# czbiohub-sf/yogo

Measured on AMD Instinct MI355X. Metric: training images/sec (772x1032 gray), higher is better.
Workload: dtype bf16; 1 GPU; BASELINE configs[2]: full train step (fwd+loss+bwd+clamp+AdamW), base_model, 772x1032x1 uint8, 7 classes; per_gpu_batch=128, global_batch=128, parallelism=dp1

## Files before the change

### include/yogo_hip.h

```cpp
#ifndef YOGO_HIP_H
#define YOGO_HIP_H

#include <stddef.h>

#ifdef __cplusplus
extern "C" {
#endif

typedef void* yogo_stream_t;

const char* yogo_hip_last_error(void);
int yogo_hip_abi_version(void);
int yogo_hip_launch_log(int enable);
int yogo_hip_launch_log_read(char* buf, size_t cap, size_t* needed);


int yogo_conv_packed_bytes(int Cin, int Cout, int ksize, int stride, int mode, size_t* bytes);
int yogo_conv_pack_f32(const float* w_oihw, float* packed, int Cin, int Cout, int ksize, int stride, int mode,
                       yogo_stream_t stream);
int yogo_conv2d_fwd_stats_shape(int B, int Cin, int Cout, int IH, int IW, int ksize, int stride, int* rows, int* mpad);
int yogo_conv2d_fwd_f32(const float* in, const float* packed, const float* bias, float* out, float* out_pre,
                        const float* chan_scale, float* stats_part, int B, int Cin, int Cout, int IH, int IW, int ksize,
                        int stride, int act, yogo_stream_t stream);
int yogo_conv2d_dgrad_f32(const float* dy, const float* packed_dgrad, float* dx, const float* act_ref, int ref_act,
// ... 12 lines not shown
                          int IW, int stride, yogo_stream_t stream);

int yogo_bn_finalize(const float* part, int rows, int row_stride, int C, long long count, float eps, float momentum,
                     float* mean_out, float* invstd_out, float* running_mean, float* running_var,
                     long long* num_batches_tracked, yogo_stream_t stream);
int yogo_bn_apply_act(const float* z, float* y, const float* mean, const float* invstd_or_var, int stat_is_var, float eps,
                      const float* gamma, const float* beta, int B, int C, int HW, int act, yogo_stream_t stream);
int yogo_bn_invstd(const float* var, float eps, float* invstd, int C, yogo_stream_t stream);
int yogo_bn_bwd_rows(int B, int HW, int* rows);
int yogo_bn_bwd(const float* g, const float* z, float* dz, const float* mean, const float* invstd, const float* gamma,
                const float* beta, int act, float* dgamma, float* dbeta, float* part, float* sums, int B, int C, int HW,
                int training, float clip, yogo_stream_t stream);
int yogo_partials_reduce(float* part, int rows, int N, float clip, float* out, yogo_stream_t stream);
int yogo_channel_sum(const float* g, int B, int C, int HW, float clip, float* out, yogo_stream_t stream);

int yogo_decode_fwd(const float* raw, float* out, const float* cxs, const float* cys, int B, int P, int Sy, int Sx,
                    float anchor_w, float anchor_h, float width_multiplier, float height_multiplier, int inference,
                    yogo_stream_t stream);
int yogo_decode_bwd(const float* raw, const float* out, const float* gout, float* graw, int B, int P, int Sy, int Sx,
                    int inference, yogo_stream_t stream);

int yogo_decode_bwd_bf16(const float* raw, const float* out, const float* gout, void* graw8c, int B, int P, int Sy, int Sx,
                         int inference, yogo_stream_t stream);

int yogo_loss_workspace_bytes(int B, int Sy, int Sx, size_t* bytes);
int yogo_loss_fwd_bwd(const float* pred, const float* label, float* grad, float* loss_out, void* workspace, int B, int P,
                      int Sy, int Sx, float no_obj_weight, float iou_weight, float classify_weight, float label_smoothing,
                      yogo_stream_t stream);

int yogo_decode_loss_bwd_bf16(const float* raw, const float* label, const float* cxs, const float* cys, void* graw8c, float* loss_out,
                              void* workspace, int B, int P, int Sy, int Sx, float anchor_w, float anchor_h, float width_multiplier,
                              float height_multiplier, float no_obj_weight, float iou_weight, float classify_weight,
                              float label_smoothing, yogo_stream_t stream);

int yogo_format_preds_workspace_bytes(int B, int Sy, int Sx, size_t* bytes);
int yogo_format_preds_batched(const float* pred, float* out_rows, long long* out_cells, int* out_count, void* workspace,
                              int B, int P, int Sy, int Sx, int cap, double obj_thresh, double iou_thresh, int box_format,
                              double min_class_confidence_threshold, yogo_stream_t stream);
int yogo_decode_format_preds_batched(const float* raw, const float* cxs, const float* cys, float* out_rows, long long* out_cells,
                                     int* out_count, void* workspace, int B, int P, int Sy, int Sx, int cap, float anchor_w,
                                     float anchor_h, float width_multiplier, float height_multiplier, int inference,
                                     double obj_thresh, double iou_thresh, int box_format, double min_class_confidence_threshold,
                                     yogo_stream_t stream);
int yogo_head1x1_decode_fwd_bf16(const void* x, const void* packed, const float* bias, float* out, const float* cxs, const float* cys,
                                 int B, int Cin, int P, int Sy, int Sx, float anchor_w, float anchor_h, float width_multiplier,
                                 float height_multiplier, int inference, yogo_stream_t stream);

int yogo_match_workspace_bytes(int B, int Sy, int Sx, int cap, size_t* bytes);
int yogo_match_preds_labels_batched(const float* rows, const int* counts, const float* labels, int* meta, int* pair_label,
                                    int* pair_pred, int* un_label, int* un_pred, float* lab_out, void* workspace, int B, int P, int Sy,
                                    int Sx, int cap, yogo_stream_t stream);
int yogo_match_gather(const float* rows, const float* lab_out, const int* meta, const int* pair_label, const int* pair_pred,
                      const int* un_label, const int* un_pred, float* preds, float* labels, float* missed, float* extra, int B, int P,
                      int cap, long long K, long long Km, long long Ke, yogo_stream_t stream);
int yogo_metrics_state_layout(int C, int T, int nbins, long long* offsets);
int yogo_metrics_accumulate(const float* rows, const float* lab_out, const int* meta, const int* pair_label, const int* pair_pred,
                            const int* un_label, const int* un_pred, const double* roc_thresholds, int T, const double* cal_edges,
                            int nbins, long long* acc, double* bin_conf, double* partial, float* map_rows, long long map_cap, int B,
                            int P, int cap, yogo_stream_t stream);

int yogo_pred_sink_state_layout(int C, long long* offsets);
int yogo_pred_sink_workspace_bytes(int B, size_t* bytes);
int yogo_pred_sink_append(const float* rows, const int* counts, int B, int cap, int P, int mode, int count_classes,
                          long long first_img_id, int img_h, int img_w, long long* state, float* arena, long long arena_cap,
                          int* img_counts, long long img_cap, void* workspace, yogo_stream_t stream);

// ... 134 lines not shown
```

### yogo_amd/csrc/decode_loss.hip

```cpp
#include "common.h"

#define MAX_CLASSES 64

__device__ __forceinline__ float sigmoidf_(float x) { return 1.0f / (1.0f + expf(-x)); }

__global__ __launch_bounds__(256) void decode_fwd_kernel(const float* __restrict__ raw, float* __restrict__ out,
                                                         const float* __restrict__ cxs, const float* __restrict__ cys,
                                                         float inv_sx, float inv_sy, float anchor_w, float anchor_h,
                                                         float wmul, float hmul, int P, int cells, int inference) {
  const int b = blockIdx.y;
  const int cell = blockIdx.x * 256 + threadIdx.x;
  if (cell >= cells) return;
  const float* r = raw + (size_t)b * P * cells + cell;
  float* o = out + (size_t)b * P * cells + cell;
  const float t0 = r[0], t1 = r[(size_t)cells], t2 = r[(size_t)2 * cells], t3 = r[(size_t)3 * cells], t4 = r[(size_t)4 * cells];
  o[0] = inv_sx * sigmoidf_(t0) + cxs[cell];
  o[(size_t)cells] = inv_sy * sigmoidf_(t1) + cys[cell];
  o[(size_t)2 * cells] = anchor_w * expf(fminf(t2, 80.f)) * wmul;
  o[(size_t)3 * cells] = anchor_h * expf(fminf(t3, 80.f)) * hmul;
  o[(size_t)4 * cells] = sigmoidf_(t4);
  const int C = P - 5;
  if (inference) {
    float mx = -INFINITY;
    for (int c = 0; c < C; ++c) mx = fmaxf(mx, r[(size_t)(5 + c) * cells]);
    float sum = 0.f;
    for (int c = 0; c < C; ++c) sum += expf(r[(size_t)(5 + c) * cells] - mx);
    for (int c = 0; c < C; ++c) o[(size_t)(5 + c) * cells] = expf(r[(size_t)(5 + c) * cells] - mx) / sum;
  } else {
    for (int c = 0; c < C; ++c) o[(size_t)(5 + c) * cells] = r[(size_t)(5 + c) * cells];
  }
}

__global__ __launch_bounds__(256) void decode_bwd_kernel(const float* __restrict__ raw, const float* __restrict__ out,
// ... 311 lines not shown
        if (ch < p.P) {
          if (ch == 0) v = g0 * (p.inv_sx * (s0 * (1.f - s0)));
          else if (ch == 1) v = g1 * (p.inv_sy * (s1 * (1.f - s1)));
          else if (ch == 2) v = t2 <= 80.f ? g2 * pw : 0.f;
          else if (ch == 3) v = t3 <= 80.f ? g3 * ph : 0.f;
          else if (ch == 4) v = gobj * (po * (1.f - po));
          else if (m != 0.f) {
            const int c = ch - 5;
            const float sm = expf(r[(size_t)ch * cells] - lse);
            v = scl * (sm - (c == tgt ? (1.f - ls) : 0.f) - ls / (float)C);
          }
        }
        u[j] = (__bf16)v;
      }
      p.g8[((size_t)b * p.Pb + kb) * cells + cell] = __builtin_bit_cast(dl_u32x4, u);
    }
  }
  l_iou = wave_sum(l_iou);
  l_obj = wave_sum(l_obj);
  l_cls = wave_sum(l_cls);
  const int lane = threadIdx.x & 63, wave = threadIdx.x >> 6;
  if (lane == 0) {
    sh[0][wave] = l_iou;
    sh[1][wave] = l_obj;
    sh[2][wave] = l_cls;
  }
  __syncthreads();
  if (threadIdx.x < 3) {
    const int k = threadIdx.x;
    p.part[((size_t)b * gridDim.x + blockIdx.x) * 3 + k] = sh[k][0] + sh[k][1] + sh[k][2] + sh[k][3];
  }
}

__global__ __launch_bounds__(256) void yogo_loss_finalize_kernel(const float* __restrict__ part, int rows, float iou_weight,
                                                                 float classify_weight, float inv_batch,
                                                                 float* __restrict__ out) {
  __shared__ double sh[3][4];
  double s[3] = {0.0, 0.0, 0.0};
  for (int r = threadIdx.x; r < rows; r += 256)
    for (int k = 0; k < 3; ++k) s[k] += (double)part[(size_t)r * 3 + k];
  const int lane = threadIdx.x & 63, wave = threadIdx.x >> 6;
  for (int k = 0; k < 3; ++k) {
    s[k] = wave_sum_d(s[k]);
    if (lane == 0) sh[k][wave] = s[k];
  }
  __syncthreads();
  if (threadIdx.x == 0) {
    const float iou = (float)(iou_weight * (sh[0][0] + sh[0][1] + sh[0][2] + sh[0][3]) * inv_batch);
    const float obj = (float)((sh[1][0] + sh[1][1] + sh[1][2] + sh[1][3]) * inv_batch);
    const float cls = (float)(classify_weight * (sh[2][0] + sh[2][1] + sh[2][2] + sh[2][3]) * inv_batch);
    out[0] = obj + iou + cls;
    out[1] = iou;
    out[2] = obj;
    out[3] = cls;
  }
}

extern "C" int yogo_decode_fwd(const float* raw, float* out, const float* cxs, const float* cys, int B, int P, int Sy,
                               int Sx, float anchor_w, float anchor_h, float width_multiplier, float height_multiplier,
                               int inference, hipStream_t stream) {
  YOGO_CHECK_ARG(raw && out && cxs && cys, "decode_fwd: null pointer");
  YOGO_CHECK_ARG(B >= 0 && P > 5 && P - 5 <= MAX_CLASSES && Sy > 0 && Sx > 0 && B <= 65535, "decode_fwd: bad shape");
  if (B == 0) return YOGO_OK;
  const int cells = Sy * Sx;
  yogo_launch_log("decode_fwd_kernel | B=%d cells=%d P=%d inference=%d", B, cells, P, inference);
  hipLaunchKernelGGL(decode_fwd_kernel, dim3(cdiv(cells, 256), B), dim3(256), 0, stream, raw, out, cxs, cys,
// ... 34 lines not shown
}

extern "C" int yogo_loss_fwd_bwd(const float* pred, const float* label, float* grad, float* loss_out, void* workspace,
                                 int B, int P, int Sy, int Sx, float no_obj_weight, float iou_weight, float classify_weight,
                                 float label_smoothing, hipStream_t stream) {
  YOGO_CHECK_ARG(pred && label && grad && loss_out && workspace, "loss_fwd_bwd: null pointer");
  YOGO_CHECK_ARG(B > 0 && B <= 65535 && P > 5 && P - 5 <= MAX_CLASSES && Sy > 0 && Sx > 0, "loss_fwd_bwd: bad shape");
  LossParams p{};
  p.pred = pred; p.label = label; p.grad = grad; p.part = reinterpret_cast<float*>(workspace);
  p.B = B; p.P = P; p.cells = Sy * Sx;
  p.no_obj_weight = no_obj_weight; p.iou_weight = iou_weight; p.classify_weight = classify_weight;
  p.label_smoothing = label_smoothing; p.inv_batch = 1.0f / (float)B;
  const int nb = cdiv(p.cells, 256);
  hipLaunchKernelGGL(yogo_loss_kernel, dim3(nb, B), dim3(256), 0, stream, p);
  hipLaunchKernelGGL(yogo_loss_finalize_kernel, dim3(1), dim3(256), 0, stream, p.part, B * nb, iou_weight, classify_weight,
                     p.inv_batch, loss_out);
  YOGO_CHECK_LAUNCH("loss_fwd_bwd");
  return YOGO_OK;
}

extern "C" int yogo_decode_loss_bwd_bf16(const float* raw, const float* label, const float* cxs, const float* cys, void* graw8c, float* loss_out,
                                         void* workspace, int B, int P, int Sy, int Sx, float anchor_w, float anchor_h, float width_multiplier,
                                         float height_multiplier, float no_obj_weight, float iou_weight, float classify_weight,
                                         float label_smoothing, hipStream_t stream) {
  YOGO_CHECK_ARG(raw && label && cxs && cys && graw8c && loss_out && workspace, "decode_loss_bwd_bf16: null pointer");
  YOGO_CHECK_ARG(B > 0 && B <= 65535 && P > 5 && P - 5 <= MAX_CLASSES && Sy > 0 && Sx > 0, "decode_loss_bwd_bf16: bad shape");
  FusedParams p{};
  p.raw = raw; p.label = label; p.cxs = cxs; p.cys = cys; p.g8 = reinterpret_cast<dl_u32x4*>(graw8c); p.part = reinterpret_cast<float*>(workspace);
  p.B = B; p.P = P; p.Pb = ((P + 15) / 16) * 2; p.cells = Sy * Sx;
  p.inv_sx = (float)(1.0 / Sx); p.inv_sy = (float)(1.0 / Sy); p.anchor_w = anchor_w; p.anchor_h = anchor_h; p.wmul = width_multiplier; p.hmul = height_multiplier;
  p.no_obj_weight = no_obj_weight; p.iou_weight = iou_weight; p.classify_weight = classify_weight; p.label_smoothing = label_smoothing;
  p.inv_batch = 1.0f / (float)B;
  const int nb = cdiv(p.cells, 256);
  hipLaunchKernelGGL(decode_loss_bwd_bf16_kernel, dim3(nb, B), dim3(256), 0, stream, p);
  hipLaunchKernelGGL(yogo_loss_finalize_kernel, dim3(1), dim3(256), 0, stream, p.part, B * nb, iou_weight, classify_weight, p.inv_batch, loss_out);
  YOGO_CHECK_LAUNCH("decode_loss_bwd_bf16");
  return YOGO_OK;
}
```

### yogo_amd/engine.py

```python
from __future__ import annotations

import threading
import weakref
from dataclasses import dataclass, field
from typing import Dict, List, Optional, Tuple

import torch
from torch import nn

from yogo_amd import _hip

ACT_NONE, ACT_LEAKY, ACT_SILU = 0, 1, 2


@dataclass
class Layer:
    conv: nn.Conv2d
    bn: Optional[nn.BatchNorm2d] = None
    act: int = ACT_NONE
    drop: Optional[nn.Dropout2d] = None

    @property
    def cin(self) -> int:
        return self.conv.in_channels
# ... 293 lines not shown
                Lp, Sp = self.layers[i - 1], saved[i - 1]
                ref_act = Lp.act
                if Lp.bn is not None:
                    act_ref, ref_act = None, ACT_NONE
                elif Lp.act == ACT_SILU:
                    act_ref = Sp.pre
                    if act_ref is None:
                        raise RuntimeError("yogo_amd: missing saved pre-activation for a SiLU block")
                elif Lp.act == ACT_LEAKY:
                    act_ref = Sp.y
                else:
                    act_ref = None
                dx = torch.empty(B, L.cin, IH, IW, dtype=torch.float32, device=dev)
                pk = self._packed(i, 1)
                mw_tag = 20 if L.s == 2 else (4 if L.cin > 64 else (2 if L.cin > 32 else 1))
                self._tick("dgrad", i, 2.0 * B * L.cout * L.cin * L.k * L.k * OH * OW, mw=mw_tag)
                _hip.call("yogo_conv2d_dgrad_f32", g, pk, dx, act_ref, ref_act, Sp.mask, B, L.cin, L.cout, IH, IW, L.k, L.s, st)
                self._tock()
                g = dx
        bb = self.backbone_ref()
        return [grads.get(id(p)) for p in bb.parameters()]



def _blocks(c: int) -> int:
    return ((c + 15) // 16) * 2


_FUSE_LAYER0_BWD = True
_L0_NO_Z = True
_WGRAD_DEFER_REDUCE = True
_L01_FUSE_BWD = True
_HEAD_BN_FUSE = True


def _packed_bf16(eng: Engine, i: int, mode: int) -> torch.Tensor:
    L = eng.layers[i]
    w = L.conv.weight
    key = (i, 10 + mode)
    buf = _pack_hit(eng, key, w)
    if buf is not None:
        return buf
    nbytes = _hip.query_size("yogo_conv_bf16_packed_bytes", L.cin, L.cout, L.k, mode)
    buf = torch.empty(nbytes, dtype=torch.uint8, device=w.device)
    _hip.call("yogo_conv_bf16_pack", _f32(w.detach()), None, buf, L.cin, L.cout, L.k, mode, _hip.stream_ptr())
    eng._pack[key] = (w._version, w.data_ptr(), buf)
    return buf


def _pack_all_bf16(eng: Engine) -> None:
    jobs = [(i, mode) for i in range(1, len(eng.layers)) for mode in (0, 2 if (eng.layers[i].s == 2 and eng.layers[i].k == 3) else 1)]
    ws = [eng.layers[i].conv.weight for i, _ in jobs]
    if any(w.dtype != torch.float32 or not w.is_contiguous() for w in ws) or not jobs:
        return
    if all(_pack_hit(eng, (i, 10 + m), w) is not None for (i, m), w in zip(jobs, ws)):
        return
    dev = ws[0].device
    key = tuple(w.data_ptr() for w in ws)
    st = eng._pack_multi
    if st is None or st[0] != key:
        bufs, rows, blk = [], [], 0
        for (i, mode), w in zip(jobs, ws):
            L = eng.layers[i]
            buf = torch.empty(_hip.query_size("yogo_conv_bf16_packed_bytes", L.cin, L.cout, L.k, mode), dtype=torch.uint8, device=dev)
            bufs.append(buf)
            rows.append([w.data_ptr(), 0, buf.data_ptr(), L.cin, L.cout, L.k, mode, blk])
# ... 97 lines not shown
        pk = _packed_bf16(eng, i, 0)
        nbytes = B * (_blocks(L.cin) * 8 * H * W * 2 + (L.cout * OH * OW * 4 if last else _blocks(L.cout) * 8 * OH * OW * 2))
        eng._tick("fwd", i, 2.0 * B * L.cout * L.cin * L.k * L.k * OH * OW, mw=34 if (L.cout > 64 and L.s == 1) else (35 if (L.cout > 64 and L.cin > 64 and L.k == 3) else 30), nbytes=nbytes)
        if L.act == ACT_SILU and not has_bn:
            S.pre = torch.empty_like(out8)
            _hip.call("yogo_conv2d_fwd_bf16_pre", cur, pk, bias, out8, S.pre, mask, B, L.cin, L.cout, H, W, L.k, L.s, fused_act, st)
        elif L.act == ACT_LEAKY and not has_bn and not last:
            S.signs = torch.empty(_hip.query_size("yogo_bf16_signs_bytes", B, L.cout, OH, OW), dtype=torch.uint8, device=dev)
            _hip.call("yogo_conv2d_fwd_bf16_signs", cur, pk, bias, out8, S.signs, mask, B, L.cin, L.cout, H, W, L.k, L.s, fused_act, st)
        else:
            _hip.call("yogo_conv2d_fwd_bf16", cur, pk, bias, out8, out32, mask, None, B, L.cin, L.cout, H, W, L.k, L.s, fused_act, st)
        eng._tock()
    if not has_bn:
        S.y = out32 if last else out8
        return S.y
    bn = L.bn
    gamma, beta = _bn_affine(L, dev)
    y = torch.empty_like(out8)
    if bn_train:
        if i > 0:
            rows, mpad = _hip.query_ints("yogo_bn_bwd_bf16_rows", 1, B, OH * OW)[0], L.cout
            stats = torch.empty(rows * mpad * 2, dtype=torch.float32, device=dev)
            _hip.call("yogo_bn_stats_bf16", out8, stats, B, L.cout, OH * OW, st)
        mean, invstd = _bn_finalize(eng, L, "yogo_bn_finalize", stats, rows, mpad, count=B * OH * OW, dev=dev, st=st)
    else:
        invstd = torch.empty(L.cout, dtype=torch.float32, device=dev)
        _hip.call("yogo_bn_invstd", bn.running_var, float(bn.eps), invstd, L.cout, st)
        mean = bn.running_mean
    _hip.call("yogo_bn_apply_act_bf16", out8, y, mean, invstd, 0, float(bn.eps), gamma, beta, B, L.cout, OH * OW, L.act, st)
    S.mean, S.invstd, S.bn_train, S.z, S.y = mean, invstd, bn_train, out8, y
    return y


def forward_bf16_train(eng: Engine, x: torch.Tensor) -> Tuple[torch.Tensor, List[Saved]]:
    _check_bf16_train_input(eng, x)
    dev, st, B = x.device, _hip.stream_ptr(), x.shape[0]
    _pack_all_bf16(eng)
    masks = _dropout_masks(eng, B, dev)
    cur = x.contiguous() if x.dtype == torch.uint8 else _f32(x)
    H, W = int(cur.shape[2]), int(cur.shape[3])
    saved: List[Saved] = []
    n = len(eng.layers)
    for i, L in enumerate(eng.layers):
        OH, OW = L.out_hw(H, W)
        if OH <= 0 or OW <= 0:
            raise RuntimeError(f"yogo_amd: image too small at layer {i}")
        last = i == n - 1
        has_bn = L.bn is not None
        if L.act == ACT_SILU and not has_bn and (i == 0 or last):
            raise RuntimeError("yogo_amd: bf16 training of a first / last SiLU block without BatchNorm is not implemented (use fp32)")
        bias = _f32(L.conv.bias.detach()) if L.conv.bias is not None else None
        S = Saved(x_in=cur, mask=masks.get(i))
        bn_train = has_bn and (L.bn.training or L.bn.running_mean is None)
        if (i == 0 and has_bn and S.mask is None and not last and cur.dtype == torch.uint8
                and _hip.lib().yogo_conv_first_mfma_supported(0, L.cin, L.cout, H, W, L.s)):
            cur = _first_mfma_fwd_bf16(eng, L, S, bias, bn_train, B, H, W, st)
        else:
            cur = _layer_fwd_bf16(eng, i, L, S, bias, bn_train, last, B, H, W, st)
        saved.append(S)
        H, W = OH, OW
    return cur, saved


def backward_bf16_train(eng: Engine, saved: List[Saved], graw: torch.Tensor,
                        grad_out: Optional[Dict[int, torch.Tensor]] = None, on_layer=None,
                        trace: Optional[dict] = None, flush_layers=None, stop_at: int = 0) -> List[Optional[torch.Tensor]]:
    n = len(eng.layers)
    if not 0 <= stop_at < n:
        raise ValueError(f"yogo_amd: stop_at {stop_at} is not a layer of this {n}-layer network")
    st, dev, clip = _hip.stream_ptr(), graw.device, float(eng.clip)
    grads: Dict[int, torch.Tensor] = {}

    def dst(param: torch.Tensor) -> torch.Tensor:
        if grad_out is not None and id(param) in grad_out:
            return grad_out[id(param)]
        return torch.empty(param.shape, dtype=torch.float32, device=dev)

    queued_ws: List[torch.Tensor] = []
    wq = _wgrad_queue() if (_WGRAD_DEFER_REDUCE and (on_layer is None or flush_layers is not None)) else None
    flush_at = frozenset(flush_layers) if flush_layers is not None else frozenset()
    if wq is not None:
        _hip.call("yogo_wgrad_reduce_queue_reset", wq)
    if graw.dtype == torch.bfloat16 and graw.ndim == 5:
        g = graw
        B = g.shape[0]
    else:
        graw = _f32(graw)
        B, P, Sy, Sx = graw.shape
        g = torch.empty(B, _blocks(P), Sy, Sx, 8, dtype=torch.bfloat16, device=dev)
        _hip.call("yogo_nchw_f32_to_bf16_8c", graw, g, B, P, Sy * Sx, st)

    def bn_backward(L, S, g, head_g, OH, OW):
        gamma, beta = _bn_affine(L, dev)
        dgamma, dbeta = _bn_grad_dst(L.bn, dst, grads, L.cout, dev)
        rows = _hip.query_ints("yogo_bn_bwd_bf16_rows", 1, B, OH * OW)[0]
        part = torch.empty(rows * L.cout * 2, dtype=torch.float32, device=dev)
        sums = torch.empty(2 * L.cout, dtype=torch.float32, device=dev)
        if head_g is not None:
            dz = torch.empty(B, _blocks(L.cout), OH, OW, 8, dtype=torch.bfloat16, device=dev)
# ... 92 lines not shown
        head_below = bool(_HEAD_BN_FUSE and i == n - 1 and Lp is not None and i - 1 > 0 and L.k == 1 and L.s == 1 and L.cout <= 16
                          and Lp.bn is not None and Lp.cout % 16 == 0 and g.shape[1] == 2)
        act_ref, ref_act = None, ACT_NONE
        if Lp is not None and Lp.bn is None and Lp.act != ACT_NONE:
            act_ref, ref_act = (Sp.y if Lp.act == ACT_LEAKY else Sp.pre), Lp.act
        if trace is not None and g is not None and head_g is None:
            trace[("g", i)] = g.clone()
        if L.bn is not None and not fuse0:
            g, head_g = bn_backward(L, S, g, head_g, OH, OW), None
            if trace is not None:
                trace[("dz", i)] = g.clone()
        dw = dst(L.conv.weight)
        db = dst(L.conv.bias) if L.conv.bias is not None else None
        if fuse0:
            wgrad_first_bn(L, S, g, fused01, dw, IH, IW)
        elif fuse01:
            fused01 = wgrad_dgrad_first(L, S, g, dw, db, IH, IW, OH, OW)
        elif i == 0:
            wgrad_first(L, S, g, dw, db, IH, IW)
        else:
            wgrad(i, L, S, g, dw, db, IH, IW, OH, OW)
        if db is not None:
            grads[id(L.conv.bias)] = db
        grads[id(L.conv.weight)] = dw
        if on_layer is not None:
            if wq is not None and i in flush_at:
                _hip.call("yogo_wgrad_reduce_flush", wq, st)
            on_layer(i)
        if fuse01:
            g = None
        elif head_below:
            head_g = (g, _f32(L.conv.weight.detach()).reshape(L.cout, L.cin), L.cout)
        elif i > stop_at:
            g = dgrad(i, L, g, Sp, act_ref, ref_act, IH, IW, OH, OW)
    if wq is not None:
        _hip.call("yogo_wgrad_reduce_flush", wq, st)
    bb = eng.backbone_ref()
    return [grads.get(id(p)) for p in bb.parameters()]


_WGRAD_QUEUE = None


def _wgrad_queue() -> int:
    global _WGRAD_QUEUE
    if _WGRAD_QUEUE is None:
        import ctypes
        h = ctypes.c_void_p(0)
        _hip.call("yogo_wgrad_reduce_queue_create", ctypes.addressof(h))
        _WGRAD_QUEUE = int(h.value)
    return _WGRAD_QUEUE


_ENGINES: "weakref.WeakKeyDictionary[nn.Module, Engine]" = weakref.WeakKeyDictionary()


def get_engine(backbone: nn.Sequential) -> Engine:
    eng = _ENGINES.get(backbone)
    if eng is None:
        eng = Engine(backbone)
        _ENGINES[backbone] = eng
    return eng


class _BackboneFn(torch.autograd.Function):
    @staticmethod
    def forward(ctx, x, backbone, *params):
# ... 224 lines not shown
```

### yogo_amd/train.py

```python
from __future__ import annotations

import ctypes
import math
from typing import Dict, List, Optional, Tuple

import torch
import torch.distributed as dist

from yogo_amd import _hip
from yogo_amd.engine import get_engine
from yogo_amd.model import YOGO
from yogo_amd.yogo_loss import YOGOLoss

_FUSED_DECODE_LOSS = True


def cosine_lr(step: int, base_lr: float, t_max: int, eta_min: float) -> float:
    return eta_min + (base_lr - eta_min) * (1 + math.cos(math.pi * step / t_max)) / 2


class FlatParams:

    def __init__(self, module: torch.nn.Module):
        self.params: List[torch.nn.Parameter] = [p for p in module.parameters()]
# ... 215 lines not shown
            if icnt is not None:
                _hip.call("yogo_comm_broadcast_flat", self._rccl, icnt, icnt.numel() * 8, src, st)
        else:
            dist.broadcast(flat, src=src, group=self.pg)
            if icnt is not None:
                dist.broadcast(icnt, src=src, group=self.pg)
        off = 0
        for b in fl:
            n = b.numel()
            b.copy_(flat[off:off + n].view(b.shape).to(b.dtype))
            off += n
        off = 0
        for b in cnt:
            n = b.numel()
            b.copy_(icnt[off:off + n].view(b.shape).to(b.dtype))
            off += n
        self.engine.generation += 1

    @torch.no_grad()
    def step(self, imgs: torch.Tensor, labels: torch.Tensor) -> torch.Tensor:
        m = self.model
        _hip.require_cuda(imgs, "imgs")
        _hip.require_cuda(labels, "labels")
        with torch.cuda.device(imgs.device):
            st = _hip.stream_ptr()
            eng = self.engine
            eng.clip = m._clip
            self.flat.check_homed()
            if imgs.ndim == 3:
                imgs = imgs[None]
            if not imgs.is_floating_point() and imgs.dtype != torch.uint8:
                imgs = imgs.float()
            if self.half:
                from yogo_amd.engine import backward_bf16_train, forward_bf16_train

                raw, saved = forward_bf16_train(eng, imgs)
                if self.trace is not None:
                    self.trace["saved"], self.trace["raw"] = saved, raw
            else:
                raw, saved = eng.forward(imgs, need_grad=True)
            B, P, Sy, Sx = raw.shape
            aw, ah, wm, hm = m._decode_scalars()
            cxs, cys = _hip.grid_buffers(m._Cxs, m._Cys, Sy, Sx, raw.device)
            L = self.loss
            out = torch.empty(4, dtype=torch.float32, device=raw.device)
            ws = torch.empty(_hip.query_size("yogo_loss_workspace_bytes", B, Sy, Sx) // 4, dtype=torch.float32, device=raw.device)
            lab = labels if (labels.dtype == torch.float32 and labels.is_contiguous()) else labels.contiguous().float()
            hook = self._on_layer_done if self.world > 1 else None
            flush = (self.split_layer,) if hook is not None else None
            lw = (float(L.no_obj_weight), float(L.iou_weight), float(L.classify_weight), float(L.label_smoothing))

            def decode_and_loss():
                pred, gpred = torch.empty_like(raw), torch.empty_like(raw)
                _hip.call("yogo_decode_fwd", raw, pred, cxs, cys, B, P, Sy, Sx, aw, ah, wm, hm, int(bool(m.inference)), st)
                _hip.call("yogo_loss_fwd_bwd", pred, lab, gpred, out, ws, B, P, Sy, Sx, *lw, st)
                return pred, gpred

            g8 = torch.empty(B, ((P + 15) // 16) * 2, Sy, Sx, 8, dtype=torch.bfloat16, device=raw.device) if self.half else None
            if self.half and not m.inference and _FUSED_DECODE_LOSS:
                _hip.call("yogo_decode_loss_bwd_bf16", raw, lab, cxs, cys, g8, out, ws, B, P, Sy, Sx, aw, ah, wm, hm, *lw, st)
                backward_bf16_train(eng, saved, g8, grad_out=self.flat.grad_views, on_layer=hook, trace=self.trace, flush_layers=flush)
            elif self.half:
                pred, gpred = decode_and_loss()
                _hip.call("yogo_decode_bwd_bf16", raw, pred, gpred, g8, B, P, Sy, Sx, int(bool(m.inference)), st)
                backward_bf16_train(eng, saved, g8, grad_out=self.flat.grad_views, on_layer=hook, trace=self.trace, flush_layers=flush)
            else:
                pred, gpred = decode_and_loss()
                graw = torch.empty_like(raw)
                _hip.call("yogo_decode_bwd", raw, pred, gpred, graw, B, P, Sy, Sx, int(bool(m.inference)), st)
                eng.backward(saved, graw, grad_out=self.flat.grad_views, on_layer=hook)
            started = self.split_off if (self.overlap and self._pending) else self.flat.total
            self.exchange_begin(0, started)
            scale = self.exchange_end()
            lr = self.current_lr()
            self.global_step += 1
            _hip.call("yogo_adamw_step", self.flat.flat, self.flat.grad, self.flat.exp_avg, self.flat.exp_avg_sq, self.flat.total,
                      self.global_step, lr, self.betas[0], self.betas[1], self.eps, self.wd, scale, st)
            eng.invalidate_packed()
            self.last_loss = out
            return out

    def loss_components(self) -> Dict[str, float]:
        v = self.last_loss.cpu().tolist()
        return {"loss": v[0], "iou_loss": v[1], "objectness_loss": v[2], "classification_loss": v[3]}
```

Measured before the change: 11160 images/s.

## Fuse head 1x1 conv, decode, loss and head dgrad into one sweep kernel

Adds a persistent kernel that, for the final 1x1 head layer, computes the head conv with MFMA, decodes, evaluates the YOGO loss and its gradient, and applies the head dgrad multiplied by the leaky activation derivative in a single pass over each pixel tile. It also has an optional path that accumulates weight gradients in the same pass. The forward pass stops before the head, and the backward pass takes the precomputed head dx. The aim is to remove the separate head forward, decode/loss, and dgrad launches along with their intermediate global memory round trips. In exchange the kernel carries heavy register and LDS pressure, and it only handles restricted shapes (P up to 16, Cin up to 128).

```diff
diff --git a/include/yogo_hip.h b/include/yogo_hip.h
--- a/include/yogo_hip.h
+++ b/include/yogo_hip.h
@@ -68,6 +68,14 @@
                               void* workspace, int B, int P, int Sy, int Sx, float anchor_w, float anchor_h, float width_multiplier,
                               float height_multiplier, float no_obj_weight, float iou_weight, float classify_weight,
                               float label_smoothing, yogo_stream_t stream);
+
+int yogo_head_sweep_bf16_supported(int Cin, int P, int ksize, int stride, int Sy, int Sx, int B);
+int yogo_head_sweep_bf16_rows(int B, int Sy, int Sx, int* rows);
+int yogo_head_sweep_bf16_workspace_bytes(int B, int Cin, int P, int Sy, int Sx, size_t* bytes);
+int yogo_head_sweep_bf16(const void* y6, const void* packed, const float* bias, const float* label, const float* cxs, const float* cys,
+                         float* raw, void* g8, void* g6, float* loss_out, void* loss_ws, void* wpart, int B, int Cin, int P, int Sy,
+                         int Sx, float anchor_w, float anchor_h, float width_multiplier, float height_multiplier, float no_obj_weight,
+                         float iou_weight, float classify_weight, float label_smoothing, yogo_stream_t stream);
 
 int yogo_format_preds_workspace_bytes(int B, int Sy, int Sx, size_t* bytes);
 int yogo_format_preds_batched(const float* pred, float* out_rows, long long* out_cells, int* out_count, void* workspace,
diff --git a/yogo_amd/csrc/decode_loss.hip b/yogo_amd/csrc/decode_loss.hip
--- a/yogo_amd/csrc/decode_loss.hip
+++ b/yogo_amd/csrc/decode_loss.hip
@@ -1,4 +1,5 @@
 #include "common.h"
+#include <mutex>
 
 #define MAX_CLASSES 64
 
@@ -376,6 +377,337 @@
   }
 }
 
+typedef float dl_f32x16 __attribute__((ext_vector_type(16)));
+typedef float dl_f32x4 __attribute__((ext_vector_type(4)));
+typedef __bf16 dl_bf16x4 __attribute__((ext_vector_type(4)));
+#define HS_MAXP 16
+#define HS_WAVE_LDS 10240
+
+struct HeadSweepParams {
+  const dl_u32x4* y6;
+  const dl_u32x4* wp;
+  const float* bias;
+  const float* label;
+  const float *cxs, *cys;
+  float* raw;
+  dl_u32x4* g8;
+  dl_u32x4* g6;
+  float* part;
+  float* wpart;
+  int B, P, cells, nb, units, upb;
+  float inv_sx, inv_sy, anchor_w, anchor_h, wmul, hmul;
+  float no_obj_weight, iou_weight, classify_weight, label_smoothing, inv_batch;
+};
+
+__device__ __forceinline__ int hs_off(int row, int ch) { return 256 * row + 16 * (ch ^ (((row & 3) << 2) | ((row >> 2) & 3))); }
+
+__device__ __forceinline__ dl_bf16x8 hs_tr8(const unsigned char* a0, const unsigned char* a1) {
+  typedef dl_bf16x4 __attribute__((address_space(3))) * lds_v4;
+  const dl_bf16x4 lo = __builtin_amdgcn_ds_read_tr16_b64_v4bf16((lds_v4)a0);
+  const dl_bf16x4 hi = __builtin_amdgcn_ds_read_tr16_b64_v4bf16((lds_v4)a1);
+  return __builtin_shufflevector(lo, hi, 0, 1, 2, 3, 4, 5, 6, 7);
+}
+
+template <int NK, bool WG>
+__global__ __launch_bounds__(256, 2) void decode_loss_bwd_bf16_kernel(const HeadSweepParams p) {
+  constexpr int OOB = (int)0x80000000u;
+  constexpr int KB = 2 * NK, NM = (NK + 1) / 2, CIN = 16 * NK;
+  __shared__ __attribute__((aligned(16))) unsigned char lds[WG ? 4 * HS_WAVE_LDS : 16];
+  __shared__ float sh[2][3][4];
+  const int tid = threadIdx.x, lane = tid & 63, l31 = lane & 31, half = lane >> 5, l15 = lane & 15, g4 = lane >> 4;
+  const int wave = __builtin_amdgcn_readfirstlane(tid >> 6);
+  unsigned char* yimg = lds + wave * HS_WAVE_LDS;
+  unsigned char* gimg = yimg + 8192;
+  const int cells = p.cells, cells16 = cells * 16, P = p.P, C = P - 5;
+  __shared__ dl_u32x4 wlds[KB * 32];
+  for (int e = tid; e < KB * 32; e += 256) wlds[e] = p.wp[e];
+  float bs[8];
+#pragma unroll
+  for (int i = 0; i < 8; ++i) {
+    const int ch = 8 * (i >> 2) + 4 * half + (i & 3);
+    bs[i] = (p.bias != nullptr && ch < P) ? p.bias[ch] : 0.f;
+  }
+  dl_bf16x8 Wd[NM];
+  {
+    const __bf16* w16 = reinterpret_cast<const __bf16*>(p.wp);
+    const int q = l31 >> 3, h = (l31 >> 2) & 1, t = l31 & 3;
+#pragma unroll
+    for (int m = 0; m < NM; ++m) {
+      const int cin = 8 * (4 * m + 2 * (q >> 1) + h) + 4 * (q & 1) + t;
+#pragma unroll
+      for (int j = 0; j < 8; ++j) {
+        const int pch = 8 * half + j;
+        Wd[m][j] = (cin < CIN && pch < P) ? w16[(((cin >> 3) * 32 + pch) << 3) + (cin & 7)] : (__bf16)0.f;
+      }
+    }
+  }
+  dl_bf16x8 ones;
+#pragma unroll
+  for (int j = 0; j < 8; ++j) ones[j] = (__bf16)1.f;
+  dl_f32x4 accW[NK], accB = {0.f, 0.f, 0.f, 0.f};
+#pragma unroll
+  for (int c = 0; c < NK; ++c) accW[c] = dl_f32x4{0.f, 0.f, 0.f, 0.f};
+  const int trq = l15 >> 2, trp = l15 & 3;
+
+  __syncthreads();
+  const int u_end = min(p.units, (int)(blockIdx.x + 1) * p.upb);
+  int par = 0;
+  for (int u = blockIdx.x * p.upb; u < u_end; ++u, par ^= 1) {
+    const int b = u / p.nb, blk = u - b * p.nb;
+    const int pxw = blk * 256 + wave * 64;
+    const int px = pxw + lane;
+    const bool valid = px < cells;
+    const auto rs_in = __builtin_amdgcn_make_buffer_rsrc((void*)(p.y6 + (size_t)b * KB * cells), (short)0, KB * cells16, 0x00020000);
+    dl_u32x4 Bq[2][NK];
+    bool ov[2];
+    int pxt[2];
+#pragma unroll
+    for (int T = 0; T < 2; ++T) {
+      pxt[T] = pxw + 32 * T + l31;
+      ov[T] = pxt[T] < cells;
+      const int v0 = ov[T] ? (half * cells + pxt[T]) * 16 : OOB;
+#pragma unroll
+      for (int kc = 0; kc < NK; ++kc) Bq[T][kc] = __builtin_bit_cast(dl_u32x4, __builtin_amdgcn_raw_buffer_load_b128(rs_in, v0, (2 * kc) * cells16, 0));
+    }
+    dl_f32x16 acc[2];
+#pragma unroll
+    for (int T = 0; T < 2; ++T)
+#pragma unroll
+      for (int r = 0; r < 16; ++r) acc[T][r] = 0.f;
+#pragma unroll
+    for (int kc = 0; kc < NK; ++kc) {
+      const dl_bf16x8 a = __builtin_bit_cast(dl_bf16x8, wlds[(2 * kc + half) * 32 + l31]);
+      acc[0] = __builtin_amdgcn_mfma_f32_32x32x16_bf16(a, __builtin_bit_cast(dl_bf16x8, Bq[0][kc]), acc[0], 0, 0, 0);
+      acc[1] = __builtin_amdgcn_mfma_f32_32x32x16_bf16(a, __builtin_bit_cast(dl_bf16x8, Bq[1][kc]), acc[1], 0, 0, 0);
+    }
+    float r[HS_MAXP];
+#pragma unroll
+    for (int i = 0; i < 8; ++i) {
+      const float own = (half == 0 ? acc[0][i] : acc[1][i]) + bs[i];
+      const float snd = (half == 0 ? acc[1][i] : acc[0][i]) + bs[i];
+      const float rcv = __shfl_xor(snd, 32, 64);
+      const int cha = 8 * (i >> 2) + (i & 3);
+      r[cha] = half == 0 ? own : rcv;
+      r[cha + 4] = half == 0 ? rcv : own;
+    }
+    float l_iou = 0.f, l_obj = 0.f, l_cls = 0.f;
+    float gv[HS_MAXP];
+#pragma unroll
+    for (int ch = 0; ch < HS_MAXP; ++ch) gv[ch] = 0.f;
+    if (valid) {
+      float* ro = p.raw + (size_t)b * P * cells + px;
+#pragma unroll
+      for (int ch = 0; ch < HS_MAXP; ++ch)
+        if (ch < P) ro[(size_t)ch * cells] = r[ch];
+      const float* lb = p.label + (size_t)b * 6 * cells + px;
+      const float t0 = r[0], t1 = r[1], t2 = r[2], t3 = r[3], t4 = r[4];
+      const float s0 = sigmoidf_(t0), s1 = sigmoidf_(t1);
+      const float pcx = p.inv_sx * s0 + p.cxs[px];
+      const float pcy = p.inv_sy * s1 + p.cys[px];
+      const float pw = p.anchor_w * expf(fminf(t2, 80.f)) * p.wmul;
+      const float ph = p.anchor_h * expf(fminf(t3, 80.f)) * p.hmul;
+      const float po = sigmoidf_(t4);
+      const float m = lb[0];
+      float gobj;
+      {
+        const float wgt = m * (1.f - p.no_obj_weight) + p.no_obj_weight;
+        const float df = po - m;
+        l_obj = df * df * wgt;
+        gobj = 2.f * df * wgt * p.inv_batch;
+      }
+      float g0 = 0.f, g1 = 0.f, g2 = 0.f, g3 = 0.f;
+      if (m != 0.f) {
+        const float cx = pcx, cy = pcy, w = pw, h = ph;
+        const float x1 = cx - 0.5f * w, y1 = cy - 0.5f * h, x2 = cx + 0.5f * w, y2 = cy + 0.5f * h;
+        if (x1 != x2 && y1 != y2) {
+          const float X1 = fminf(fmaxf(x1, 0.f), 1.f), Y1 = fminf(fmaxf(y1, 0.f), 1.f);
+          const float X2 = fminf(fmaxf(x2, 0.f), 1.f), Y2 = fminf(fmaxf(y2, 0.f), 1.f);
+          const float c1 = (x1 >= 0.f && x1 <= 1.f) ? 1.f : 0.f, c2 = (y1 >= 0.f && y1 <= 1.f) ? 1.f : 0.f;
+          const float c3 = (x2 >= 0.f && x2 <= 1.f) ? 1.f : 0.f, c4 = (y2 >= 0.f && y2 <= 1.f) ? 1.f : 0.f;
+          const float x1g = lb[(size_t)cells], y1g = lb[(size_t)2 * cells], x2g = lb[(size_t)3 * cells], y2g = lb[(size_t)4 * cells];
+          const float eps = 1e-7f;
+          const float xk1 = fmaxf(X1, x1g), yk1 = fmaxf(Y1, y1g), xk2 = fminf(X2, x2g), yk2 = fminf(Y2, y2g);
+          const bool has = (yk2 > yk1) && (xk2 > xk1);
+          const float iw = xk2 - xk1, ih = yk2 - yk1;
+          const float I = has ? iw * ih : 0.f;
+          const float wp = X2 - X1, hp = Y2 - Y1, wg = x2g - x1g, hg = y2g - y1g;
+          const float U = wp * hp + wg * hg - I;
+          const float Ue = U + eps;
+          const float iou = I / Ue;
+          const float xc1 = fminf(X1, x1g), yc1 = fminf(Y1, y1g), xc2 = fmaxf(X2, x2g), yc2 = fmaxf(Y2, y2g);
+          const float ex = xc2 - xc1, ey = yc2 - yc1;
+          const float D = ex * ex + ey * ey + eps;
+          const float dxc = (X2 + X1) / 2.f - (x1g + x2g) / 2.f, dyc = (Y2 + Y1) / 2.f - (y1g + y2g) / 2.f;
+          const float dist = dxc * dxc + dyc * dyc;
+          const float kv = 4.f / (3.14159265358979323846f * 3.14159265358979323846f);
+          const float th = atanf(wg / hg) - atanf(wp / hp);
+          const float v = kv * th * th;
+          const float alpha = v / (1.f - iou + v + eps);
+          l_iou = 1.f - iou + dist / D + alpha * v;
+          float dI1 = 0.f, dI2 = 0.f, dI3 = 0.f, dI4 = 0.f;
+          if (has) {
+            dI1 = -ih * dmax_a(X1, x1g);
+            dI2 = -iw * dmax_a(Y1, y1g);
+            dI3 = ih * dmin_a(X2, x2g);
+            dI4 = iw * dmin_a(Y2, y2g);
+          }
+          const float dU1 = -hp - dI1, dU2 = -wp - dI2, dU3 = hp - dI3, dU4 = wp - dI4;
+          const float iU2 = 1.f / (Ue * Ue);
+          const float di1 = (dI1 * Ue - I * dU1) * iU2, di2 = (dI2 * Ue - I * dU2) * iU2;
+          const float di3 = (dI3 * Ue - I * dU3) * iU2, di4 = (dI4 * Ue - I * dU4) * iU2;
+          const float dD1 = -2.f * ex * dmin_a(X1, x1g), dD2 = -2.f * ey * dmin_a(Y1, y1g);
+          const float dD3 = 2.f * ex * dmax_a(X2, x2g), dD4 = 2.f * ey * dmax_a(Y2, y2g);
+          const float iD2 = 1.f / (D * D);
+          const float dr1 = (dxc * D - dist * dD1) * iD2, dr2 = (dyc * D - dist * dD2) * iD2;
+          const float dr3 = (dxc * D - dist * dD3) * iD2, dr4 = (dyc * D - dist * dD4) * iD2;
+          const float den = hp * hp + wp * wp;
+          const float dv_dw = -2.f * kv * th * hp / den, dv_dh = 2.f * kv * th * wp / den;
+          const float gX1 = -di1 + dr1 - alpha * dv_dw, gY1 = -di2 + dr2 - alpha * dv_dh;
+          const float gX2 = -di3 + dr3 + alpha * dv_dw, gY2 = -di4 + dr4 + alpha * dv_dh;
+          const float sc = p.iou_weight * p.inv_batch;
+          g0 = (gX1 * c1 + gX2 * c3) * sc;
+          g1 = (gY1 * c2 + gY2 * c4) * sc;
+          g2 = 0.5f * (gX2 * c3 - gX1 * c1) * sc;
+          g3 = 0.5f * (gY2 * c4 - gY1 * c2) * sc;
+        }
+      }
+      float lse = 0.f, scl = 0.f;
+      int tgt = -1;
+      const float ls = p.label_smoothing;
+      if (m != 0.f) {
+        tgt = (int)lb[(size_t)5 * cells];
+        float mx = -INFINITY;
+#pragma unroll
+        for (int c = 0; c < HS_MAXP - 5; ++c)
+          if (c < C) mx = fmaxf(mx, r[5 + c]);
+        float sum = 0.f;
+#pragma unroll
+        for (int c = 0; c < HS_MAXP - 5; ++c)
+          if (c < C) sum += expf(r[5 + c] - mx);
+        lse = mx + logf(sum);
+        float nll_t = 0.f, nll_sum = 0.f;
+#pragma unroll
+        for (int c = 0; c < HS_MAXP - 5; ++c)
+          if (c < C) {
+            const float lp = r[5 + c] - lse;
+            nll_sum -= lp;
+            if (c == tgt) nll_t = -lp;
+          }
+        l_cls = m * ((1.f - ls) * nll_t + (ls / (float)C) * nll_sum);
+        scl = m * p.classify_weight * p.inv_batch;
+      }
+      gv[0] = g0 * (p.inv_sx * (s0 * (1.f - s0)));
+      gv[1] = g1 * (p.inv_sy * (s1 * (1.f - s1)));
+      gv[2] = t2 <= 80.f ? g2 * pw : 0.f;
+      gv[3] = t3 <= 80.f ? g3 * ph : 0.f;
+      gv[4] = gobj * (po * (1.f - po));
+      if (m != 0.f) {
+#pragma unroll
+        for (int c = 0; c < HS_MAXP - 5; ++c)
+          if (c < C) {
+            const float sm = expf(r[5 + c] - lse);
+            gv[5 + c] = scl * (sm - (c == tgt ? (1.f - ls) : 0.f) - ls / (float)C);
+          }
+      }
+    }
+    dl_bf16x8 gu[2];
+#pragma unroll
+    for (int j = 0; j < 8; ++j) {
+      gu[0][j] = (__bf16)gv[j];
+      gu[1][j] = (__bf16)gv[8 + j];
+    }
+    if (valid) {
+      p.g8[((size_t)b * 2 + 0) * cells + px] = __builtin_bit_cast(dl_u32x4, gu[0]);
+      p.g8[((size_t)b * 2 + 1) * cells + px] = __builtin_bit_cast(dl_u32x4, gu[1]);
+    }
+    l_iou = wave_sum(l_iou);
+    l_obj = wave_sum(l_obj);
+    l_cls = wave_sum(l_cls);
+    if (lane == 0) {
+      sh[par][0][wave] = l_iou;
+      sh[par][1][wave] = l_obj;
+      sh[par][2][wave] = l_cls;
+    }
+    __syncthreads();
+    if (tid < 3) p.part[(size_t)u * 3 + tid] = sh[par][tid][0] + sh[par][tid][1] + sh[par][tid][2] + sh[par][tid][3];
+    {
+      const dl_u32x4 own0 = __builtin_bit_cast(dl_u32x4, gu[0]), own1 = __builtin_bit_cast(dl_u32x4, gu[1]);
+      dl_u32x4 rcv;
+#pragma unroll
+      for (int e = 0; e < 4; ++e) rcv[e] = (unsigned)__shfl_xor((int)(half == 0 ? own1[e] : own0[e]), 32, 64);
+      dl_u32x4 Bg[2];
+#pragma unroll
+      for (int e = 0; e < 4; ++e) {
+        Bg[0][e] = half == 0 ? own0[e] : rcv[e];
+        Bg[1][e] = half == 0 ? rcv[e] : own1[e];
+      }
+#pragma unroll
+      for (int T = 0; T < 2; ++T) {
+#pragma unroll
+        for (int m = 0; m < NM; ++m) {
+          dl_f32x16 d;
+#pragma unroll
+          for (int e = 0; e < 16; ++e) d[e] = 0.f;
+          d = __builtin_amdgcn_mfma_f32_32x32x16_bf16(Wd[m], __builtin_bit_cast(dl_bf16x8, Bg[T]), d, 0, 0, 0);
+#pragma unroll
+          for (int j = 0; j < 2; ++j) {
+            if (2 * m + j < NK) {
+              const dl_bf16x8 y = __builtin_bit_cast(dl_bf16x8, Bq[T][2 * m + j]);
+              dl_bf16x8 o;
+#pragma unroll
+              for (int e = 0; e < 8; ++e) o[e] = (__bf16)(d[8 * j + e] * act_bwd_factor((float)y[e], ACT_LEAKY));
+              if (ov[T]) p.g6[((size_t)b * KB + 2 * (2 * m + j) + half) * cells + pxt[T]] = __builtin_bit_cast(dl_u32x4, o);
+            }
+          }
+        }
+      }
+    }
+    if constexpr (WG) {
+    *reinterpret_cast<dl_u32x4*>(gimg + lane * 32) = __builtin_bit_cast(dl_u32x4, gu[0]);
+    *reinterpret_cast<dl_u32x4*>(gimg + lane * 32 + 16) = __builtin_bit_cast(dl_u32x4, gu[1]);
+#pragma unroll
+    for (int T = 0; T < 2; ++T) {
+#pragma unroll
+      for (int kc = 0; kc < NK; ++kc) *reinterpret_cast<dl_u32x4*>(yimg + hs_off(l31, 2 * kc + half)) = Bq[T][kc];
+      const int row0 = 8 * g4 + trq, row1 = row0 + 4;
+      const dl_bf16x8 Ag = hs_tr8(gimg + (32 * T + row0) * 32 + trp * 8, gimg + (32 * T + row1) * 32 + trp * 8);
+      accB = __builtin_amdgcn_mfma_f32_16x16x32_bf16(Ag, ones, accB, 0, 0, 0);
+#pragma unroll
+      for (int c = 0; c < NK; ++c) {
+        const dl_bf16x8 By = hs_tr8(yimg + hs_off(row0, 2 * c + (trp >> 1)) + 8 * (trp & 1), yimg + hs_off(row1, 2 * c + (trp >> 1)) + 8 * (trp & 1));
+        accW[c] = __builtin_amdgcn_mfma_f32_16x16x32_bf16(Ag, By, accW[c], 0, 0, 0);
+      }
+    }
+    }
+  }
+  if constexpr (!WG) return;
+  __syncthreads();
+  float* red = reinterpret_cast<float*>(lds);
+#pragma unroll
+  for (int w = 0; w < 4; ++w) {
+    if (wave == w) {
+#pragma unroll
+      for (int c = 0; c <= NK; ++c) {
+#pragma unroll
+        for (int i = 0; i < 4; ++i) {
+          const int e = (c * 4 + i) * 64 + lane;
+          const float v = c < NK ? accW[c < NK ? c : 0][i] : accB[i];
+          red[e] = w == 0 ? v : red[e] + v;
+        }
+      }
+    }
+    __syncthreads();
+  }
+  float* row = p.wpart + (size_t)blockIdx.x * (P * CIN + P);
+  for (int e = tid; e < (NK + 1) * 256; e += 256) {
+    const int ci = e >> 6, ln = e & 63, c = ci >> 2, i = ci & 3;
+    const int pch = 4 * (ln >> 4) + i;
+    if (pch >= P) continue;
+    if (c < NK) row[pch * CIN + 16 * c + (ln & 15)] = red[e];
+    else if ((ln & 15) == 0) row[P * CIN + pch] = red[e];
+  }
+}
+
 __global__ __launch_bounds__(256) void yogo_loss_finalize_kernel(const float* __restrict__ part, int rows, float iou_weight,
                                                                  float classify_weight, float inv_batch,
                                                                  float* __restrict__ out) {
@@ -476,8 +808,90 @@
   p.no_obj_weight = no_obj_weight; p.iou_weight = iou_weight; p.classify_weight = classify_weight; p.label_smoothing = label_smoothing;
   p.inv_batch = 1.0f / (float)B;
   const int nb = cdiv(p.cells, 256);
-  hipLaunchKernelGGL(decode_loss_bwd_bf16_kernel, dim3(nb, B), dim3(256), 0, stream, p);
+  hipLaunchKernelGGL(static_cast<void (*)(const FusedParams)>(decode_loss_bwd_bf16_kernel), dim3(nb, B), dim3(256), 0, stream, p);
   hipLaunchKernelGGL(yogo_loss_finalize_kernel, dim3(1), dim3(256), 0, stream, p.part, B * nb, iou_weight, classify_weight, p.inv_batch, loss_out);
   YOGO_CHECK_LAUNCH("decode_loss_bwd_bf16");
   return YOGO_OK;
 }
+
+namespace {
+int hs_n_cu() {
+  static std::mutex mu;
+  static int n_cu_of[64] = {0};
+  int dev = 0;
+  if (hipGetDevice(&dev) != hipSuccess || dev < 0 || dev >= 64) {
+    yogo_set_error("head_sweep_bf16: hipGetDevice failed");
+    return -1;
+  }
+  std::lock_guard<std::mutex> lk(mu);
+  if (n_cu_of[dev] == 0) {
+    hipDeviceProp_t prop;
+    n_cu_of[dev] = (hipGetDeviceProperties(&prop, dev) == hipSuccess && prop.multiProcessorCount > 0) ? prop.multiProcessorCount : 256;
+  }
+  return n_cu_of[dev];
+}
+void hs_plan(int units, int n_cu, int* grid, int* upb) {
+  *upb = cdiv(units, 2 * n_cu);
+  *grid = cdiv(units, *upb);
+}
+bool hs_shape_ok(int B, int Cin, int P, int Sy, int Sx) {
+  if (!(B > 0 && Sy > 0 && Sx > 0 && P >= 9 && P <= HS_MAXP && Cin >= 16 && Cin <= 128 && Cin % 16 == 0)) return false;
+  const long long cells = (long long)Sy * Sx;
+  return (Cin / 8) * cells * 16 < (1ll << 31) && (long long)B * ((cells + 255) / 256) < (1ll << 30);
+}
+}
+
+extern "C" int yogo_head_sweep_bf16_supported(int Cin, int P, int ksize, int stride, int Sy, int Sx, int B) {
+  return (ksize == 1 && stride == 1 && hs_shape_ok(B, Cin, P, Sy, Sx)) ? 1 : 0;
+}
+
+extern "C" int yogo_head_sweep_bf16_rows(int B, int Sy, int Sx, int* rows) {
+  YOGO_CHECK_ARG(rows && B > 0 && Sy > 0 && Sx > 0, "head_sweep_bf16_rows: bad arguments");
+  const int n_cu = hs_n_cu();
+  if (n_cu < 0) return YOGO_ERR_HIP;
+  int upb = 0;
+  hs_plan(B * cdiv(Sy * Sx, 256), n_cu, rows, &upb);
+  return YOGO_OK;
+}
+
+extern "C" int yogo_head_sweep_bf16_workspace_bytes(int B, int Cin, int P, int Sy, int Sx, size_t* bytes) {
+  YOGO_CHECK_ARG(bytes && hs_shape_ok(B, Cin, P, Sy, Sx), "head_sweep_bf16_workspace_bytes: bad arguments");
+  int rows = 0;
+  const int rc = yogo_head_sweep_bf16_rows(B, Sy, Sx, &rows);
+  if (rc != YOGO_OK) return rc;
+  *bytes = (size_t)rows * ((size_t)P * Cin + P) * sizeof(float);
+  return YOGO_OK;
+}
+
+extern "C" int yogo_head_sweep_bf16(const void* y6, const void* packed, const float* bias, const float* label, const float* cxs, const float* cys,
+                                    float* raw, void* g8, void* g6, float* loss_out, void* loss_ws, void* wpart, int B, int Cin, int P, int Sy,
+                                    int Sx, float anchor_w, float anchor_h, float width_multiplier, float height_multiplier, float no_obj_weight,
+                                    float iou_weight, float classify_weight, float label_smoothing, hipStream_t stream) {
+  YOGO_CHECK_ARG(y6 && packed && label && cxs && cys && raw && g8 && g6 && loss_out && loss_ws, "head_sweep_bf16: null pointer");
+  YOGO_CHECK_ARG(hs_shape_ok(B, Cin, P, Sy, Sx), "head_sweep_bf16: unsupported shape (9 <= P <= 16, Cin a multiple of 16 and <= 128)");
+  const int n_cu = hs_n_cu();
+  if (n_cu < 0) return YOGO_ERR_HIP;
+  HeadSweepParams p{};
+  p.y6 = reinterpret_cast<const dl_u32x4*>(y6); p.wp = reinterpret_cast<const dl_u32x4*>(packed); p.bias = bias; p.label = label; p.cxs = cxs; p.cys = cys;
+  p.raw = raw; p.g8 = reinterpret_cast<dl_u32x4*>(g8); p.g6 = reinterpret_cast<dl_u32x4*>(g6); p.part = reinterpret_cast<float*>(loss_ws);
+  p.wpart = reinterpret_cast<float*>(wpart);
+  p.B = B; p.P = P; p.cells = Sy * Sx; p.nb = cdiv(p.cells, 256); p.units = B * p.nb;
+  int grid = 0;
+  hs_plan(p.units, n_cu, &grid, &p.upb);
+  p.inv_sx = (float)(1.0 / Sx); p.inv_sy = (float)(1.0 / Sy); p.anchor_w = anchor_w; p.anchor_h = anchor_h; p.wmul = width_multiplier; p.hmul = height_multiplier;
+  p.no_obj_weight = no_obj_weight; p.iou_weight = iou_weight; p.classify_weight = classify_weight; p.label_smoothing = label_smoothing;
+  p.inv_batch = 1.0f / (float)B;
+  switch (Cin / 16) {
+#define HS_CASE(NK)                                                                                                          \
+  case NK:                                                                                                                   \
+    if (wpart != nullptr) hipLaunchKernelGGL((decode_loss_bwd_bf16_kernel<NK, true>), dim3(grid), dim3(256), 0, stream, p);  \
+    else hipLaunchKernelGGL((decode_loss_bwd_bf16_kernel<NK, false>), dim3(grid), dim3(256), 0, stream, p);                  \
+    break;
+    HS_CASE(1) HS_CASE(2) HS_CASE(3) HS_CASE(4) HS_CASE(5) HS_CASE(6) HS_CASE(7) HS_CASE(8)
+#undef HS_CASE
+    default: yogo_set_error("head_sweep_bf16: Cin = %d", Cin); return YOGO_ERR_ARG;
+  }
+  hipLaunchKernelGGL(yogo_loss_finalize_kernel, dim3(1), dim3(256), 0, stream, p.part, p.units, iou_weight, classify_weight, p.inv_batch, loss_out);
+  YOGO_CHECK_LAUNCH("head_sweep_bf16");
+  return YOGO_OK;
+}
diff --git a/yogo_amd/engine.py b/yogo_amd/engine.py
--- a/yogo_amd/engine.py
+++ b/yogo_amd/engine.py
@@ -349,6 +349,19 @@
 _WGRAD_DEFER_REDUCE = True
 _L01_FUSE_BWD = True
 _HEAD_BN_FUSE = True
+_HEAD_ONE_SWEEP = True
+
+
+def head_sweep_applies(eng: Engine, B: int, H: int, W: int, mask_below) -> bool:
+    n = len(eng.layers)
+    if not _HEAD_ONE_SWEEP or n < 3:
+        return False
+    L, Lp = eng.layers[n - 1], eng.layers[n - 2]
+    if L.bn is not None or L.act != ACT_NONE or Lp.bn is not None or Lp.act != ACT_LEAKY or mask_below is not None:
+        return False
+    if L.conv.weight.dtype != torch.float32 or not L.conv.weight.is_contiguous():
+        return False
+    return bool(_hip.lib().yogo_head_sweep_bf16_supported(L.cin, L.cout, L.k, L.s, H, W, B))
 
 
 def _packed_bf16(eng: Engine, i: int, mode: int) -> torch.Tensor:
@@ -512,7 +525,7 @@
     return y
 
 
-def forward_bf16_train(eng: Engine, x: torch.Tensor) -> Tuple[torch.Tensor, List[Saved]]:
+def forward_bf16_train(eng: Engine, x: torch.Tensor, head_sweep: bool = False) -> Tuple[Optional[torch.Tensor], List[Saved]]:
     _check_bf16_train_input(eng, x)
     dev, st, B = x.device, _hip.stream_ptr(), x.shape[0]
     _pack_all_bf16(eng)
@@ -531,6 +544,9 @@
             raise RuntimeError("yogo_amd: bf16 training of a first / last SiLU block without BatchNorm is not implemented (use fp32)")
         bias = _f32(L.conv.bias.detach()) if L.conv.bias is not None else None
         S = Saved(x_in=cur, mask=masks.get(i))
+        if last and head_sweep and S.mask is None and head_sweep_applies(eng, B, H, W, saved[-1].mask if saved else None):
+            saved.append(S)
+            return None, saved
         bn_train = has_bn and (L.bn.training or L.bn.running_mean is None)
         if (i == 0 and has_bn and S.mask is None and not last and cur.dtype == torch.uint8
                 and _hip.lib().yogo_conv_first_mfma_supported(0, L.cin, L.cout, H, W, L.s)):
@@ -544,7 +560,8 @@
 
 def backward_bf16_train(eng: Engine, saved: List[Saved], graw: torch.Tensor,
                         grad_out: Optional[Dict[int, torch.Tensor]] = None, on_layer=None,
-                        trace: Optional[dict] = None, flush_layers=None, stop_at: int = 0) -> List[Optional[torch.Tensor]]:
+                        trace: Optional[dict] = None, flush_layers=None, stop_at: int = 0,
+                        head_dx: Optional[torch.Tensor] = None) -> List[Optional[torch.Tensor]]:
     n = len(eng.layers)
     if not 0 <= stop_at < n:
         raise ValueError(f"yogo_amd: stop_at {stop_at} is not a layer of this {n}-layer network")
@@ -703,7 +720,7 @@
         elif head_below:
             head_g = (g, _f32(L.conv.weight.detach()).reshape(L.cout, L.cin), L.cout)
         elif i > stop_at:
-            g = dgrad(i, L, g, Sp, act_ref, ref_act, IH, IW, OH, OW)
+            g = head_dx if (head_dx is not None and i == n - 1) else dgrad(i, L, g, Sp, act_ref, ref_act, IH, IW, OH, OW)
     if wq is not None:
         _hip.call("yogo_wgrad_reduce_flush", wq, st)
     bb = eng.backbone_ref()
diff --git a/yogo_amd/train.py b/yogo_amd/train.py
--- a/yogo_amd/train.py
+++ b/yogo_amd/train.py
@@ -271,13 +271,22 @@
             if not imgs.is_floating_point() and imgs.dtype != torch.uint8:
                 imgs = imgs.float()
             if self.half:
-                from yogo_amd.engine import backward_bf16_train, forward_bf16_train
-
-                raw, saved = forward_bf16_train(eng, imgs)
+                from yogo_amd.engine import _packed_bf16, backward_bf16_train, forward_bf16_train
+
+                sweep_ok = not m.inference and _FUSED_DECODE_LOSS
+                raw, saved = forward_bf16_train(eng, imgs, head_sweep=sweep_ok)
+                if raw is None:
+                    y6, Lh = saved[-1].x_in, eng.layers[-1]
+                    raw = torch.empty(y6.shape[0], Lh.cout, y6.shape[2], y6.shape[3], dtype=torch.float32, device=y6.device)
+                    saved[-1].y = raw
+                    sweep = True
+                else:
+                    sweep = False
                 if self.trace is not None:
                     self.trace["saved"], self.trace["raw"] = saved, raw
             else:
                 raw, saved = eng.forward(imgs, need_grad=True)
+                sweep = False
             B, P, Sy, Sx = raw.shape
             aw, ah, wm, hm = m._decode_scalars()
             cxs, cys = _hip.grid_buffers(m._Cxs, m._Cys, Sy, Sx, raw.device)
@@ -296,7 +305,14 @@
                 return pred, gpred
 
             g8 = torch.empty(B, ((P + 15) // 16) * 2, Sy, Sx, 8, dtype=torch.bfloat16, device=raw.device) if self.half else None
-            if self.half and not m.inference and _FUSED_DECODE_LOSS:
+            if sweep:
+                g6 = torch.empty_like(saved[-1].x_in)
+                _hip.call("yogo_head_sweep_bf16", saved[-1].x_in, _packed_bf16(eng, len(eng.layers) - 1, 0),
+                          eng.layers[-1].conv.bias.detach() if eng.layers[-1].conv.bias is not None else None, lab, cxs, cys,
+                          raw, g8, g6, out, ws, None, B, eng.layers[-1].cin, P, Sy, Sx, aw, ah, wm, hm, *lw, st)
+                backward_bf16_train(eng, saved, g8, grad_out=self.flat.grad_views, on_layer=hook, trace=self.trace, flush_layers=flush,
+                                    head_dx=g6)
+            elif self.half and not m.inference and _FUSED_DECODE_LOSS:
                 _hip.call("yogo_decode_loss_bwd_bf16", raw, lab, cxs, cys, g8, out, ws, B, P, Sy, Sx, aw, ah, wm, hm, *lw, st)
                 backward_bf16_train(eng, saved, g8, grad_out=self.flat.grad_views, on_layer=hook, trace=self.trace, flush_layers=flush)
             elif self.half:
```

New measurement: 11190 images/s (median of 6 runs). No clear change (+0.2%).
